# cwerner/deadtrees

Measured on AMD Instinct MI355X. Metric: 512x512 RGB tiles/sec (train fwd+bwd), higher is better.
Workload: dtype f32; 1 GPU; configs[1]: reference U-Net (smp Unet/resnet34 topology) fp32 train step, batch 32/GPU, 512x512x3 tiles, GDICE+FOCAL, clip 0.5, Adam 3e-4; global_batch=32, tile=512, parallelism=dp1

## Files before the change

deadtrees_amd/csrc/common.h:

```cpp
#pragma once
#include <hip/hip_runtime.h>
#include <stdint.h>
#include <stdio.h>
#include <stdarg.h>
#include <type_traits>

#include "../../include/deadtrees_hip.h"

typedef float f32x16 __attribute__((ext_vector_type(16)));
typedef float f32x4 __attribute__((ext_vector_type(4)));
typedef float f32x2 __attribute__((ext_vector_type(2)));
typedef unsigned u32x2 __attribute__((ext_vector_type(2)));
typedef unsigned u32x4 __attribute__((ext_vector_type(4)));
typedef __bf16 bf16x8 __attribute__((ext_vector_type(8)));
typedef __bf16 bf16x4 __attribute__((ext_vector_type(4)));
typedef __bf16 bf16x2 __attribute__((ext_vector_type(2)));
typedef const void __attribute__((address_space(1)))* dt_gptr;
typedef void __attribute__((address_space(3)))* dt_lptr;

void dt_set_error(const char* fmt, ...);

#define DT_REQUIRE(cond, ...)            \
  do {                                   \
    if (!(cond)) {                       \
// ... 7 lines not shown
    hipError_t e__ = hipGetLastError();                                          \
    if (e__ != hipSuccess) {                                                     \
      dt_set_error("%s:%d launch failed: %s", __FILE__, __LINE__, hipGetErrorString(e__)); \
      return DT_EHIP;                                                            \
    }                                                                            \
  } while (0)

static inline int dt_cdiv(int64_t a, int64_t b) { return (int)((a + b - 1) / b); }

__device__ __forceinline__ float wave_sum(float v) {
#pragma unroll
  for (int o = 32; o > 0; o >>= 1) v += __shfl_xor(v, o, 64);
  return v;
}
__device__ __forceinline__ double wave_sum_d(double v) {
#pragma unroll
  for (int o = 32; o > 0; o >>= 1) v += __shfl_xor(v, o, 64);
  return v;
}

int dt_reduce_rows_launch(const float* in, float* out, int planes, int P, int N, int RB, hipStream_t st);
static inline int dt_reduce_rows_out(int P, int RB) { return (P + RB - 1) / RB; }

template <int K, int N, class F>
__device__ __forceinline__ void dt_static_for(F&& f) {
  if constexpr (K < N) {
    f(std::integral_constant<int, K>{});
    dt_static_for<K + 1, N>(f);
  }
}

__device__ __forceinline__ void dt_dma16(const void* g, void* l) {
  __builtin_amdgcn_global_load_lds((dt_gptr)g, (dt_lptr)l, 16, 0, 0);
}

__device__ __forceinline__ unsigned xcd_remap(unsigned id, unsigned n) {
  const unsigned q = n >> 3, r = n & 7u, xcd = id & 7u, idx = id >> 3;
  const unsigned base = xcd < r ? xcd * (q + 1) : r * (q + 1) + (xcd - r) * q;
  return base + idx;
}

extern "C" int dt_conv2d_n16_supported(const dt_conv_desc* d);
int dt_conv2d_n16_launch(const dt_conv_desc* d, const float* src0, const float* w, float* out, float* stats,
                         const float* in_scale, const float* in_shift, hipStream_t st,
                         const dt_bn_bwd_fuse* fuse = nullptr);
extern "C" int dt_conv2d_wgrad_n16_supported(const dt_conv_desc* d);
// ... 15 lines not shown
```

deadtrees_amd/csrc/conv_bf16.hip:

```cpp
#include "conv_host.h"


#include "conv_bf16.h"

#define BF_CK 32
#define BF_TF_MAXC 512
#define BF_NARROW_CIN 32

template <int KS, int STRIDE, int TW, int TPX>
struct BfGeom {
  static constexpr int TH = TPX / TW;
  static constexpr int LS = (KS == 1) ? 1 : STRIDE;
  static constexpr int GS = (KS == 1) ? STRIDE : 1;
  static constexpr int HALO_H = (TH - 1) * LS + KS;
  static constexpr int HALO_W = (TW - 1) * LS + KS;
  static constexpr int TAPS = KS * KS;
};

template <int KS, int STRIDE, int TW, int TN, int CK, int MT, bool TF>
__global__ __launch_bounds__(256, (KS == 3 && STRIDE == 2) ? 1 : 2) void conv_fwd_bf16_kernel(const ConvBfArgs a) {
  constexpr int TPX = 128 * MT;
  using G = BfGeom<KS, STRIDE, TW, TPX>;
  constexpr int BF_PITCH = CK + 8, SEG = CK / 8, ROWS_IT = 256 / SEG;
  constexpr int NT = TN / 32;
// ... 1091 lines not shown
             "wgrad_bf16: ksize/stride (%d,%d) unsupported", d->ksize, d->stride);
  DT_REQUIRE((d->C0 & 7) == 0 && (d->C1 & 7) == 0 && (d->Cout & 7) == 0, "wgrad_bf16: channels must be multiples of 8");
  DT_REQUIRE(d->mode0 >= 0 && d->mode0 <= 1, "wgrad_bf16: mode0");
  return dt_conv_validate_out(d, "wgrad_bf16");
}

extern "C" size_t dt_conv2d_wgrad_bf16_workspace(const dt_conv_desc* d) {
  if (wb_validate(d) != DT_OK) return 0;
  int tw, ks, T, cib, cob;
  wb_cfg(d, &tw, &ks, &T, &cib, &cob);
  const size_t E = (size_t)d->ksize * d->ksize * (d->C0 + d->C1) * d->Cout;
  size_t need = (size_t)ks * E * sizeof(float);
  if (dt_wgrad_bf16_narrow_supported(d)) {
    const size_t n3 = dt_wgrad_bf16_narrow_workspace(d);
    if (n3 > need) need = n3;
  }
  if (wb_use_dma() && dt_wgrad_bf16_dma_supported(d)) {
    const size_t n2 = dt_wgrad_bf16_dma_workspace(d);
    if (n2 > need) need = n2;
  }
  return need;
}

__global__ __launch_bounds__(256) void wgrad_bf16_final_kernel(const float* __restrict__ ws, float* __restrict__ dw,
                                                               int parts, int64_t E) {
  __shared__ f32x4 sh[256];
  const int q = threadIdx.x & 15, rl = threadIdx.x >> 4;
  const int64_t E4 = E >> 2, e4 = (int64_t)blockIdx.x * 16 + q;
  f32x4 a0 = {0.f, 0.f, 0.f, 0.f}, a1 = a0, a2 = a0, a3 = a0;
  if (e4 < E4) {
    const f32x4* src = reinterpret_cast<const f32x4*>(ws) + e4;
    int p = rl;
    for (; p + 48 < parts; p += 64) {
      const f32x4 v0 = src[(size_t)p * E4], v1 = src[(size_t)(p + 16) * E4];
      const f32x4 v2 = src[(size_t)(p + 32) * E4], v3 = src[(size_t)(p + 48) * E4];
      a0 += v0; a1 += v1; a2 += v2; a3 += v3;
    }
    for (; p < parts; p += 16) a0 += src[(size_t)p * E4];
  }
  sh[threadIdx.x] = (a0 + a1) + (a2 + a3);
  __syncthreads();
  if (rl == 0 && e4 < E4) {
    double t[4] = {0.0, 0.0, 0.0, 0.0};
    for (int i = 0; i < 16; ++i) {
      const f32x4 v = sh[i * 16 + q];
#pragma unroll
      for (int k = 0; k < 4; ++k) t[k] += (double)v[k];
    }
    reinterpret_cast<f32x4*>(dw)[e4] = f32x4{(float)t[0], (float)t[1], (float)t[2], (float)t[3]};
  }
}

template <int KS, int STRIDE, int TW>
static int wb_launch(const WgradBfArgs& a, int grid, hipStream_t st) {
  const bool narrow = a.C0 + a.C1 <= 32 && a.Cout <= 32;
  if (narrow) {
    if constexpr (KS == 3 && STRIDE == 1) {
      if (a.in_scale != nullptr)
        hipLaunchKernelGGL((conv_wgrad_bf16_kernel<KS, STRIDE, TW, true, 32>), dim3(grid), dim3(256), 0, st, a);
      else
        hipLaunchKernelGGL((conv_wgrad_bf16_kernel<KS, STRIDE, TW, false, 32>), dim3(grid), dim3(256), 0, st, a);
      DT_LAUNCH_CHECK();
      return DT_OK;
    }
  }
  if (a.in_scale != nullptr)
    hipLaunchKernelGGL((conv_wgrad_bf16_kernel<KS, STRIDE, TW, true, 64>), dim3(grid), dim3(256), 0, st, a);
  else
    hipLaunchKernelGGL((conv_wgrad_bf16_kernel<KS, STRIDE, TW, false, 64>), dim3(grid), dim3(256), 0, st, a);
  DT_LAUNCH_CHECK();
  return DT_OK;
}

extern "C" int dt_conv2d_wgrad_bf16(const dt_conv_desc* d, const void* src0, const void* src1, const void* dy,
                                    float* dw_hwio, float* workspace, size_t workspace_bytes, const float* in_scale,
                                    const float* in_shift, void* stream) {
  int rc = wb_validate(d);
  if (rc != DT_OK) return rc;
  DT_REQUIRE(src0 && dy && dw_hwio && workspace, "wgrad_bf16: null pointer");
  DT_REQUIRE(d->C1 == 0 || src1, "wgrad_bf16: src1 missing");
  DT_REQUIRE((in_scale == nullptr) == (in_shift == nullptr), "wgrad_bf16: in_scale/in_shift must come together");
  DT_REQUIRE(workspace_bytes >= dt_conv2d_wgrad_bf16_workspace(d), "wgrad_bf16: workspace too small");
  hipStream_t st = (hipStream_t)stream;
  const int64_t E = (int64_t)d->ksize * d->ksize * (d->C0 + d->C1) * d->Cout;
  if (dt_wgrad_bf16_narrow_supported(d)) {
    const int parts = dt_wgrad_bf16_narrow_launch(d, src0, dy, workspace, in_scale, in_shift, st);
    if (parts < 0) return parts;
    hipLaunchKernelGGL(wgrad_bf16_final_kernel, dim3((unsigned)((E / 4 + 15) / 16)), dim3(256), 0, st, workspace, dw_hwio,
                       parts, E);
    DT_LAUNCH_CHECK();
    return DT_OK;
  }
  if (in_scale == nullptr && wb_use_dma() && dt_wgrad_bf16_dma_supported(d)) {
    const int parts = dt_wgrad_bf16_dma_launch(d, src0, src1, dy, workspace, st);
    if (parts < 0) return parts;
    hipLaunchKernelGGL(wgrad_bf16_final_kernel, dim3((unsigned)((E / 4 + 15) / 16)), dim3(256), 0, st, workspace, dw_hwio,
                       parts, E);
    DT_LAUNCH_CHECK();
    return DT_OK;
  }
  WgradBfArgs a;
  int tw;
  wb_cfg(d, &tw, &a.ksplit, &a.T, &a.ci_blocks, &a.co_blocks);
  a.src0 = (const __bf16*)src0; a.src1 = (const __bf16*)src1; a.dy = (const __bf16*)dy; a.ws = workspace;
  a.in_scale = in_scale; a.in_shift = in_shift;
  a.B = d->B; a.Hin = d->Hin; a.Win = d->Win; a.C0 = d->C0; a.C1 = d->C1; a.mode0 = d->mode0;
  a.Ho = d->Ho; a.Wo = d->Wo; a.Cout = d->Cout; a.pad = d->pad;
  a.tiles_x = dt_cdiv(d->Wo, tw); a.tiles_y = dt_cdiv(d->Ho, 128 / tw);
  const int grid = a.ci_blocks * a.co_blocks * a.ksplit * (d->ksize == 4 ? 2 : 1);
  if (d->ksize == 4) {
    DT_REQUIRE(in_scale == nullptr, "wgrad_bf16: the stem takes no input transform");
    hipLaunchKernelGGL((conv_wgrad_bf16_kernel<4, 1, 32, false, 32>), dim3(grid), dim3(256), 0, st, a);
    DT_LAUNCH_CHECK();
    rc = DT_OK;
  } else if (d->ksize == 3 && d->stride == 1) rc = tw == 32 ? wb_launch<3, 1, 32>(a, grid, st) : wb_launch<3, 1, 16>(a, grid, st);
  else if (d->ksize == 3) rc = tw == 32 ? wb_launch<3, 2, 32>(a, grid, st) : wb_launch<3, 2, 16>(a, grid, st);
  else if (d->stride == 2) rc = tw == 32 ? wb_launch<1, 2, 32>(a, grid, st) : wb_launch<1, 2, 16>(a, grid, st);
  else rc = tw == 32 ? wb_launch<1, 1, 32>(a, grid, st) : wb_launch<1, 1, 16>(a, grid, st);
  if (rc != DT_OK) return rc;
  DT_REQUIRE((E & 3) == 0, "wgrad_bf16: weight tensor size must be a multiple of 4");
  const int64_t g = (E / 4 + 15) / 16;
  hipLaunchKernelGGL(wgrad_bf16_final_kernel, dim3((unsigned)g), dim3(256), 0, st, workspace, dw_hwio, a.ksplit, E);
  DT_LAUNCH_CHECK();
  return DT_OK;
}
```

deadtrees_amd/csrc/conv_wgrad.hip:

```cpp
#include "conv_host.h"

struct WgradArgs {
  const float* src0;
  const float* src1;
  const float* in_scale;
  const float* in_shift;
  const float* dy;
  const __bf16* dy_bf16;
  float* ws;
  int B, Hin, Win, C0, C1, mode0;
  int Ho, Wo, Cout, pad;
  int tiles_x, tiles_y, T;
  int ci_blocks, co_blocks, ksplit;
};

template <int KS, int STRIDE, int TW, int TPX>
struct WGeom {
  static constexpr int TH = TPX / TW;
  static constexpr int LS = (KS == 1) ? 1 : STRIDE;
  static constexpr int GS = (KS == 1) ? STRIDE : 1;
  static constexpr int HALO_H = (TH - 1) * LS + KS;
  static constexpr int HALO_W = (TW - 1) * LS + KS;
  static constexpr int TAPS = KS * KS;
};
// ... 132 lines not shown
#pragma unroll
        for (int t = 0; t < G::TAPS; ++t) {
          const int kh = t / KS, kw = t % KS;
          const float av = lx[xbase + ((yy * WK * G::LS + kh) * G::HALO_W + 2 * j * G::LS + kw) * CIW];
          acc[t] = __builtin_amdgcn_mfma_f32_32x32x2f32(av, bv, acc[t], 0, 0, 0);
        }
      }
    }
  }
  const int part = ks * WK + wk;
  const int co = co0 + wco * 32 + r;
  if (co < a.Cout) {
#pragma unroll
    for (int t = 0; t < G::TAPS; ++t) {
#pragma unroll
      for (int i = 0; i < 16; ++i) {
        const int ci = ci0 + wci * 32 + (i & 3) + 8 * (i >> 2) + 4 * s;
        if (ci < Cin) a.ws[(((size_t)part * G::TAPS + t) * Cin + ci) * a.Cout + co] = acc[t][i];
      }
    }
  }
}

__global__ __launch_bounds__(256) void wgrad_reduce_kernel(const float* __restrict__ ws, float* __restrict__ dw,
                                                           int parts, int64_t E) {
  const int64_t stride = (int64_t)gridDim.x * blockDim.x;
  for (int64_t e = (int64_t)blockIdx.x * blockDim.x + threadIdx.x; e < E; e += stride) {
    double s = 0.0;
    for (int p = 0; p < parts; ++p) s += (double)ws[(size_t)p * E + e];
    dw[e] = (float)s;
  }
}

#define STEM_TW 32
#define STEM_TH 4
__global__ __launch_bounds__(256, 2) void conv_wgrad_stem_kernel(const WgradArgs a) {
  constexpr int KS = 7, TW = STEM_TW, TH = STEM_TH;
  constexpr int HALO_H = (TH - 1) * 2 + KS, HALO_W = (TW - 1) * 2 + KS;
  constexpr int X_ELEMS = HALO_H * HALO_W * 4 + 32;
  constexpr int COW = 64;
  __shared__ __attribute__((aligned(16))) float lds[X_ELEMS + TH * TW * COW];
  float* lx = lds;
  float* ly = lds + X_ELEMS;
  const int tid = threadIdx.x, lane = tid & 63, wave = tid >> 6;
  const int s = lane >> 5, r = lane & 31;
  const int cob = blockIdx.x % a.co_blocks, ks = blockIdx.x / a.co_blocks;
  const int co0 = cob * COW;
  const int wco = wave & 1, wk = wave >> 1;
  f32x16 acc[KS];
#pragma unroll
  for (int t = 0; t < KS; ++t)
#pragma unroll
    for (int i = 0; i < 16; ++i) acc[t][i] = 0.f;
  const int Cin = a.C0;
// ... 194 lines not shown
  a.src0 = src0; a.src1 = src1; a.dy = dy; a.ws = workspace; a.in_scale = in_scale; a.in_shift = in_shift;
  a.dy_bf16 = (const __bf16*)dy_bf16;
  a.B = d->B; a.Hin = d->Hin; a.Win = d->Win; a.C0 = d->C0; a.C1 = d->C1; a.mode0 = d->mode0;
  a.Ho = d->Ho; a.Wo = d->Wo; a.Cout = d->Cout; a.pad = d->pad;
  a.tiles_x = c.tiles_x; a.tiles_y = c.tiles_y; a.T = c.T;
  a.ci_blocks = c.ci_blocks; a.co_blocks = c.co_blocks; a.ksplit = c.ksplit;
  hipStream_t st = (hipStream_t)stream;
  const int grid = c.ci_blocks * c.co_blocks * c.ksplit;
  if (c.narrow) {
    rc = dt_wgrad_n16_launch(d, src0, dy, workspace, in_scale, in_shift, st);
  } else if (c.stem) {
    hipLaunchKernelGGL(conv_wgrad_stem_kernel, dim3(grid), dim3(256), 0, st, a);
    DT_LAUNCH_CHECK();
  } else if (d->ksize == 3 && d->stride == 1) {
    rc = c.tw == 32 ? wg_dispatch<3, 1, 32>(a, c, grid, st) : wg_dispatch<3, 1, 16>(a, c, grid, st);
  } else if (d->ksize == 3 && d->stride == 2) {
    rc = c.tw == 32 ? wg_launch<3, 2, 32, 64, 1, 2>(a, grid, st) : wg_launch<3, 2, 16, 64, 1, 2>(a, grid, st);
  } else if (d->stride == 2) {
    rc = c.tw == 32 ? wg_dispatch<1, 2, 32>(a, c, grid, st) : wg_dispatch<1, 2, 16>(a, c, grid, st);
  } else {
    rc = c.tw == 32 ? wg_dispatch<1, 1, 32>(a, c, grid, st) : wg_dispatch<1, 1, 16>(a, c, grid, st);
  }
  if (rc != DT_OK) return rc;
  const float* slabs = workspace;
  int nslabs = c.parts;
  if (c.parts2 != c.parts) {
    float* stage = workspace + (size_t)c.parts * E;
    rc = dt_reduce_rows_launch(workspace, stage, 1, c.parts, (int)E, c.rb, st);
    if (rc != DT_OK) return rc;
    slabs = stage;
    nslabs = c.parts2;
  }
  const int g = dt_ew_grid(E, 256 * 8);
  hipLaunchKernelGGL(wgrad_reduce_kernel, dim3((unsigned)g), dim3(256), 0, st, slabs, dw, nslabs, E);
  DT_LAUNCH_CHECK();
  return DT_OK;
}

extern "C" int dt_conv2d_wgrad(const dt_conv_desc* d, const float* src0, const float* src1, const float* dy,
                               float* dw, float* workspace, size_t workspace_bytes, const float* in_scale,
                               const float* in_shift, void* stream) {
  return wgrad_impl(d, src0, src1, dy, nullptr, dw, workspace, workspace_bytes, in_scale, in_shift, stream);
}

extern "C" int dt_conv2d_wgrad_stem_dy_bf16(const dt_conv_desc* d, const float* src0, const void* dy_bf16, float* dw,
                                            float* workspace, size_t workspace_bytes, void* stream) {
  DT_REQUIRE(d && d->ksize == 7 && dy_bf16, "wgrad_stem_dy_bf16: 7x7 stem only");
  return wgrad_impl(d, src0, nullptr, reinterpret_cast<const float*>(dy_bf16), dy_bf16, dw, workspace, workspace_bytes,
                    nullptr, nullptr, stream);
}
```

deadtrees_amd/csrc/conv_wino_wgrad.hip:

```cpp
#include "conv_host.h"


#define WW_BUF 8192
#define WW_TF_MAXC 512
#define WW_OOB 0x80000000u
#define WW_MAX_WGS 256

struct WinoWgArgs {
  const float* src0;
  const float* src1;
  const float* dy;
  const float* in_scale;
  const float* in_shift;
  float* ws;
  int B, Hin, Win, C0, C1, mode0, Cout;
  int tiles_x, tiles_y, T;
  int ci_blocks, co_blocks, ksplit, cps;
  unsigned bytes0, bytes1, dybytes, wsbytes;
};

template <bool TF, bool CO32 = false>
__global__ __launch_bounds__(256, 1) void conv3x3_wino_wgrad_kernel(const WinoWgArgs a) {
  __shared__ __attribute__((aligned(1024))) float lds[4 * WW_BUF + (TF ? 2 * WW_TF_MAXC : 4)];
  float* Vb = lds;
// ... 251 lines not shown
  for (int c = 0; c < a.cps; c += 2) {
    asm volatile("s_waitcnt lgkmcnt(0)\n\ts_barrier" ::: "memory");
    step(S0{});
    asm volatile("s_waitcnt lgkmcnt(0)\n\ts_barrier" ::: "memory");
    step(S1{});
  }

  const __amdgpu_buffer_rsrc_t rsw = __builtin_amdgcn_make_buffer_rsrc((void*)a.ws, 0, a.wsbytes, 0x00020000);
  const unsigned lane_base = (unsigned)(((32 * wm + 4 * kh) * 64 + (CO32 ? 0 : 32 * wn) + r) * 4);
  const int wg_base = ((CO32 ? 2 * split + wn : split) * nblocks + blk) * (16 * 4096 * 4);
#pragma unroll
  for (int p = 0; p < 16; ++p) {
#pragma unroll
    for (int i = 0; i < 16; ++i) {
      const int m = (i & 3) + 8 * (i >> 2);
      const float v = acc[p][i];
      __builtin_amdgcn_raw_buffer_store_b32(__builtin_bit_cast(unsigned, v), rsw, lane_base,
                                            wg_base + (p * 4096 + m * 64) * 4, 0);
    }
    __builtin_amdgcn_sched_barrier(0);
  }
}

__global__ __launch_bounds__(256) void wino_wgrad_reduce_kernel(const float* __restrict__ ws, float* __restrict__ ws2,
                                                                int64_t n4, int ksplit, int rb) {
  const int64_t i = (int64_t)blockIdx.x * 256 + threadIdx.x;
  if (i >= n4) return;
  const int g = blockIdx.y;
  const int s0 = g * rb, s1 = s0 + rb < ksplit ? s0 + rb : ksplit;
  f32x4 s = {0.f, 0.f, 0.f, 0.f};
  for (int k = s0; k < s1; ++k) s += *reinterpret_cast<const f32x4*>(ws + ((int64_t)k * n4 + i) * 4);
  *reinterpret_cast<f32x4*>(ws2 + ((int64_t)g * n4 + i) * 4) = s;
}

__global__ __launch_bounds__(256) void wino_wgrad_final_kernel(const float* __restrict__ ws, float* __restrict__ dw,
                                                               int parts, int ci_blocks, int co_blocks, int Cin,
                                                               int Cout) {
  const int blk = blockIdx.y;
  const int e = blockIdx.x * 256 + threadIdx.x;
  const int ci = (blk / co_blocks) * 64 + (e >> 6), co = (blk % co_blocks) * 64 + (e & 63);
  if (co >= Cout) return;
  const int64_t n = (int64_t)ci_blocks * co_blocks * 16 * 4096;
  float u[16];
#pragma unroll
  for (int p = 0; p < 16; ++p) u[p] = 0.f;
  for (int k = 0; k < parts; ++k) {
    const float* src = ws + (int64_t)k * n + (int64_t)blk * 16 * 4096 + e;
#pragma unroll
    for (int p = 0; p < 16; ++p) u[p] += src[p * 4096];
  }
  float tt[12];
#pragma unroll
  for (int j = 0; j < 4; ++j) {
    tt[0 + j] = u[0 + j] + 0.5f * (u[4 + j] + u[8 + j]);
    tt[4 + j] = 0.5f * (u[4 + j] - u[8 + j]);
    tt[8 + j] = 0.5f * (u[4 + j] + u[8 + j]) + u[12 + j];
  }
#pragma unroll
  for (int i = 0; i < 3; ++i) {
    const float g0 = tt[4 * i + 0] + 0.5f * (tt[4 * i + 1] + tt[4 * i + 2]);
    const float g1 = 0.5f * (tt[4 * i + 1] - tt[4 * i + 2]);
    const float g2 = 0.5f * (tt[4 * i + 1] + tt[4 * i + 2]) + tt[4 * i + 3];
    dw[((size_t)(3 * i + 0) * Cin + ci) * Cout + co] = g0;
    dw[((size_t)(3 * i + 1) * Cin + ci) * Cout + co] = g1;
    dw[((size_t)(3 * i + 2) * Cin + ci) * Cout + co] = g2;
  }
}

struct WwCfg {
  int tiles_x, tiles_y, T, ci_blocks, co_blocks, ksplit, cps, rb, groups, parts;
};

// ... 48 lines not shown
  DT_REQUIRE((in_scale == nullptr) == (in_shift == nullptr), "wgrad_winograd: in_scale/in_shift must come together");
  DT_REQUIRE(workspace_bytes >= dt_conv2d_wgrad_winograd_workspace(d), "wgrad_winograd: workspace too small");
  const WwCfg c = ww_cfg(d);
  const size_t slab = (size_t)c.ci_blocks * c.co_blocks * 16 * 4096 * 4;
  DT_REQUIRE(slab * c.parts < 0x100000000ull, "wgrad_winograd: workspace beyond 4 GiB");
  WinoWgArgs a;
  a.src0 = src0; a.src1 = src1; a.dy = dy; a.in_scale = in_scale; a.in_shift = in_shift; a.ws = workspace;
  a.B = d->B; a.Hin = d->Hin; a.Win = d->Win; a.C0 = d->C0; a.C1 = d->C1; a.mode0 = d->mode0; a.Cout = d->Cout;
  a.tiles_x = c.tiles_x; a.tiles_y = c.tiles_y; a.T = c.T;
  a.ci_blocks = c.ci_blocks; a.co_blocks = c.co_blocks; a.ksplit = c.ksplit; a.cps = c.cps;
  const size_t px0 = (size_t)d->B * (d->mode0 ? (d->Hin / 2) * (size_t)(d->Win / 2) : (size_t)d->Hin * d->Win);
  a.bytes0 = (unsigned)(px0 * d->C0 * 4);
  a.bytes1 = (unsigned)((size_t)d->B * d->Hin * d->Win * d->C1 * 4);
  a.dybytes = (unsigned)((size_t)d->B * d->Ho * d->Wo * d->Cout * 4);
  a.wsbytes = (unsigned)(slab * c.parts);
  hipStream_t st = (hipStream_t)stream;
  dim3 g((unsigned)(c.ci_blocks * c.co_blocks * c.ksplit)), blk(256);
  if (d->Cout == 32) {
    if (in_scale != nullptr) hipLaunchKernelGGL((conv3x3_wino_wgrad_kernel<true, true>), g, blk, 0, st, a);
    else hipLaunchKernelGGL((conv3x3_wino_wgrad_kernel<false, true>), g, blk, 0, st, a);
  } else if (in_scale != nullptr) hipLaunchKernelGGL((conv3x3_wino_wgrad_kernel<true>), g, blk, 0, st, a);
  else hipLaunchKernelGGL((conv3x3_wino_wgrad_kernel<false>), g, blk, 0, st, a);
  DT_LAUNCH_CHECK();
  const float* parts_src = workspace;
  int parts = c.parts;
  if (c.rb > 1) {
    float* ws2 = workspace + slab / 4 * c.parts;
    const int64_t n4 = (int64_t)(slab / 16);
    hipLaunchKernelGGL(wino_wgrad_reduce_kernel, dim3((unsigned)dt_cdiv(n4, 256), (unsigned)c.groups), dim3(256), 0, st,
                       workspace, ws2, n4, c.parts, c.rb);
    DT_LAUNCH_CHECK();
    parts_src = ws2;
    parts = c.groups;
  }
  hipLaunchKernelGGL(wino_wgrad_final_kernel, dim3(16, (unsigned)(c.ci_blocks * c.co_blocks)), dim3(256), 0, st, parts_src,
                     dw_hwio, parts, c.ci_blocks, c.co_blocks, d->C0 + d->C1, d->Cout);
  DT_LAUNCH_CHECK();
  return DT_OK;
}
```

deadtrees_amd/csrc/elementwise.hip:

```cpp
#include "conv_host.h"
#include "views.h"

#include <math.h>

__device__ __forceinline__ void relu_mask_from_y(f32x4& g, const f32x4 yv, const f32x4 asc, const f32x4 ash) {
  const f32x4 a = yv * asc + ash;
#pragma unroll
  for (int k = 0; k < 4; ++k) g[k] = a[k] > 0.f ? g[k] : 0.f;
}
__device__ __forceinline__ void bnb_sums(const f32x4 g, const f32x4 yv, const f32x4 mu, const f32x4 is, f32x4& sg, f32x4& sx) {
  sg += g;
  sx += g * ((yv - mu) * is);
}
__device__ __forceinline__ void bnb_masked_sums(f32x4 g, const f32x4 yv, const f32x4 asc, const f32x4 ash, const f32x4 mu,
                                                const f32x4 is, f32x4& sg, f32x4& sx) {
  relu_mask_from_y(g, yv, asc, ash);
  bnb_sums(g, yv, mu, is, sg, sx);
}

__device__ __forceinline__ void bnb_store_partial_rows(const f32x4 sg, const f32x4 sx, int L, int cq, int row, int P, int C4,
                                                       float* __restrict__ red) {
  __shared__ f32x4 sh[2][256];
  const int t = threadIdx.x, rl = t / L, RL = 256 / L;
  sh[0][t] = sg;
// ... 36 lines not shown
    }
    for (; r < r1; r += RL) a0 += src[(size_t)r * N4 + cq];
  }
  sh[t] = (a0 + a1) + (a2 + a3);
  __syncthreads();
  if (rl == 0 && cq < N4) {
    f32x4 s = sh[q];
    for (int i = 1; i < RL; ++i) s += sh[i * Q + q];
    reinterpret_cast<f32x4*>(out)[((size_t)blockIdx.z * PB + blockIdx.y) * N4 + cq] = s;
  }
}

int dt_reduce_rows_launch(const float* in, float* out, int planes, int P, int N, int RB, hipStream_t st) {
  const int N4 = N / 4;
  int Q = 64;
  while (Q > N4) Q >>= 1;
  if (Q < 1) Q = 1;
  dim3 grid(dt_cdiv(N4, Q), dt_cdiv(P, RB), planes);
  hipLaunchKernelGGL(reduce_rows_kernel, grid, dim3(256), 0, st, in, out, P, N, RB, Q);
  DT_LAUNCH_CHECK();
  return DT_OK;
}

__global__ __launch_bounds__(256) void bn_finalize_kernel(const float* __restrict__ stats, int P, int C,
                                                          double count, const float* __restrict__ gamma,
                                                          const float* __restrict__ beta, float eps,
                                                          float momentum, const float* __restrict__ momentum_dev,
                                                          float* running_mean,
                                                          float* running_var, float* mean, float* invstd,
                                                          float* scale, float* shift) {
  __shared__ double red[2][16][17];
  if (momentum_dev) momentum = momentum_dev[0];
  const int cl = threadIdx.x & 15, rl = threadIdx.x >> 4;
  const int c = blockIdx.x * 16 + cl;
  double s1 = 0.0, s2 = 0.0;
  if (c < C) {
    double u1 = 0.0, u2 = 0.0, v1 = 0.0, v2 = 0.0, w1 = 0.0, w2 = 0.0;
    int p = rl;
    for (; p + 48 < P; p += 64) {
      const float a0 = stats[(size_t)p * C + c], a1 = stats[(size_t)(p + 16) * C + c];
      const float a2 = stats[(size_t)(p + 32) * C + c], a3 = stats[(size_t)(p + 48) * C + c];
      const float b0 = stats[((size_t)P + p) * C + c], b1 = stats[((size_t)P + p + 16) * C + c];
      const float b2 = stats[((size_t)P + p + 32) * C + c], b3 = stats[((size_t)P + p + 48) * C + c];
      s1 += (double)a0; u1 += (double)a1; v1 += (double)a2; w1 += (double)a3;
      s2 += (double)b0; u2 += (double)b1; v2 += (double)b2; w2 += (double)b3;
    }
    for (; p < P; p += 16) {
      s1 += (double)stats[(size_t)p * C + c];
      s2 += (double)stats[((size_t)P + p) * C + c];
    }
    s1 = (s1 + u1) + (v1 + w1);
    s2 = (s2 + u2) + (v2 + w2);
  }
  red[0][rl][cl] = s1;
  red[1][rl][cl] = s2;
  __syncthreads();
  if (rl == 0 && c < C) {
    double t1 = 0.0, t2 = 0.0;
    for (int i = 0; i < 16; ++i) {
      t1 += red[0][i][cl];
      t2 += red[1][i][cl];
    }
    const double m = t1 / count;
    double var = t2 / count - m * m;
    if (var < 0.0) var = 0.0;
    const double is = 1.0 / sqrt(var + (double)eps);
    mean[c] = (float)m;
    invstd[c] = (float)is;
    const float sc = gamma[c] * (float)is;
    scale[c] = sc;
    shift[c] = beta[c] - (float)m * sc;
    if (running_mean) {
      const double unb = count > 1.0 ? var * count / (count - 1.0) : var;
      running_mean[c] = (1.f - momentum) * running_mean[c] + momentum * (float)m;
      running_var[c] = (1.f - momentum) * running_var[c] + momentum * (float)unb;
    }
  }
}

#define BN_STAGE1_MIN_ROWS 256
#define BN_STAGE1_RB 64

extern "C" int64_t dt_bn_stats_floats(int P, int C) {
  return (int64_t)2 * P * C + (int64_t)2 * dt_reduce_rows_out(P, BN_STAGE1_RB) * C;
}

static int bn_finalize_launch(float* stats, int P, int C, double count, const float* gamma, const float* beta, float eps,
                              float momentum, const float* momentum_dev, float* running_mean, float* running_var,
                              float* mean, float* invstd, float* scale, float* shift, void* stream) {
  DT_REQUIRE(stats && gamma && beta && mean && invstd && scale && shift && P > 0 && C > 0 && count > 0,
             "bn_finalize: bad args");
  if (P > BN_STAGE1_MIN_ROWS && (C & 3) == 0) {
    const int PB = dt_reduce_rows_out(P, BN_STAGE1_RB);
    float* scratch = stats + (size_t)2 * P * C;
    int rc = dt_reduce_rows_launch(stats, scratch, 2, P, C, BN_STAGE1_RB, (hipStream_t)stream);
    if (rc != DT_OK) return rc;
    stats = scratch;
    P = PB;
  }
  hipLaunchKernelGGL(bn_finalize_kernel, dim3(dt_cdiv(C, 16)), dim3(256), 0, (hipStream_t)stream, stats, P, C,
                     count, gamma, beta, eps, momentum, momentum_dev, running_mean, running_var, mean, invstd, scale,
                     shift);
  DT_LAUNCH_CHECK();
  return DT_OK;
}

extern "C" int dt_bn_finalize(float* stats, int P, int C, double count, const float* gamma,
                              const float* beta, float eps, float momentum, float* running_mean,
                              float* running_var, float* mean, float* invstd, float* scale, float* shift,
                              void* stream) {
  return bn_finalize_launch(stats, P, C, count, gamma, beta, eps, momentum, nullptr, running_mean, running_var, mean,
                            invstd, scale, shift, stream);
}

extern "C" int dt_bn_finalize_dev(float* stats, int P, int C, double count, const float* gamma, const float* beta,
                                  float eps, const float* momentum_dev, float* running_mean, float* running_var,
                                  float* mean, float* invstd, float* scale, float* shift, void* stream) {
  DT_REQUIRE(momentum_dev && running_mean && running_var, "bn_finalize_dev: momentum_dev and running statistics required");
  return bn_finalize_launch(stats, P, C, count, gamma, beta, eps, 0.f, momentum_dev, running_mean, running_var, mean,
                            invstd, scale, shift, stream);
}

__global__ void bn_eval_affine_kernel(const float* gamma, const float* beta, const float* rm, const float* rv,
// ... 234 lines not shown
    bnb_sums(g0, y[o0], mu, is, sg0, sx0);
  }
  bnb_store_partial_rows(sg0 + sg1, sx0 + sx1, Q, cq, blockIdx.y, P, C4, red);
}

extern "C" int dt_bn_bwd_reduce(const float* dout, const float* out_act, const float* y, const float* mean,
                                const float* invstd, const float* act_scale, const float* act_shift, float* red,
                                int64_t n_pix, int C, void* stream) {
  DT_REQUIRE(dout && y && mean && invstd && red && n_pix > 0 && C > 0 && (C & 3) == 0, "bn_bwd_reduce: bad args");
  const int C4 = C / 4;
  int Q = 64;
  while (Q > C4) Q >>= 1;
  DT_REQUIRE(C4 % Q == 0, "bn_bwd_reduce: C/4 must be a power of two or a multiple of 64 (C=%d)", C);
  const int P = dt_bn_bwd_rows(n_pix, C);
  hipLaunchKernelGGL(bn_bwd_reduce_kernel, dim3(C4 / Q, P), dim3(256), 0, (hipStream_t)stream, (const f32x4*)dout,
                     (const f32x4*)out_act, (const f32x4*)y, mean, invstd, act_scale, act_shift, red, n_pix, C4, Q, P,
                     bnb_rb(n_pix));
  DT_LAUNCH_CHECK();
  return DT_OK;
}

__global__ __launch_bounds__(256) void bn_bwd_sums_kernel(const float* __restrict__ red, int P, int C,
                                                          float* __restrict__ dgamma, float* __restrict__ dbeta) {
  __shared__ double sh[2][16][17];
  const int cl = threadIdx.x & 15, rl = threadIdx.x >> 4;
  const int c = blockIdx.x * 16 + cl;
  double s1 = 0.0, s2 = 0.0;
  if (c < C) {
    double u1 = 0.0, u2 = 0.0, v1 = 0.0, v2 = 0.0, w1 = 0.0, w2 = 0.0;
    int p = rl;
    for (; p + 48 < P; p += 64) {
      const float a0 = red[(size_t)p * C + c], a1 = red[(size_t)(p + 16) * C + c];
      const float a2 = red[(size_t)(p + 32) * C + c], a3 = red[(size_t)(p + 48) * C + c];
      const float b0 = red[((size_t)P + p) * C + c], b1 = red[((size_t)P + p + 16) * C + c];
      const float b2 = red[((size_t)P + p + 32) * C + c], b3 = red[((size_t)P + p + 48) * C + c];
      s1 += (double)a0; u1 += (double)a1; v1 += (double)a2; w1 += (double)a3;
      s2 += (double)b0; u2 += (double)b1; v2 += (double)b2; w2 += (double)b3;
    }
    for (; p < P; p += 16) {
      s1 += (double)red[(size_t)p * C + c];
      s2 += (double)red[((size_t)P + p) * C + c];
    }
    s1 = (s1 + u1) + (v1 + w1);
    s2 = (s2 + u2) + (v2 + w2);
  }
  sh[0][rl][cl] = s1;
  sh[1][rl][cl] = s2;
  __syncthreads();
  if (rl == 0 && c < C) {
    double t1 = 0.0, t2 = 0.0;
    for (int i = 0; i < 16; ++i) {
      t1 += sh[0][i][cl];
      t2 += sh[1][i][cl];
    }
    dbeta[c] = (float)t1;
    dgamma[c] = (float)t2;
  }
}

int dt_bn_bwd_finish_sums(float* red, int P, int C, float* dgamma, float* dbeta, hipStream_t st) {
  if (P > BN_STAGE1_MIN_ROWS) {
    const int PB = dt_reduce_rows_out(P, BN_STAGE1_RB);
    float* scratch = red + (size_t)2 * P * C;
    int rc = dt_reduce_rows_launch(red, scratch, 2, P, C, BN_STAGE1_RB, st);
    if (rc != DT_OK) return rc;
    red = scratch;
    P = PB;
  }
  hipLaunchKernelGGL(bn_bwd_sums_kernel, dim3(dt_cdiv(C, 16)), dim3(256), 0, st, red, P, C, dgamma, dbeta);
  DT_LAUNCH_CHECK();
  return DT_OK;
}

#define BN_LD(p) __builtin_nontemporal_load(p)
__global__ __launch_bounds__(256) void bn_bwd_apply_kernel(
    const f32x4* __restrict__ dout, const f32x4* __restrict__ out_act, const f32x4* __restrict__ y,
    const float* __restrict__ mean, const float* __restrict__ invstd, const float* __restrict__ gamma,
    const float* __restrict__ dgamma, const float* __restrict__ dbeta, const float* __restrict__ act_scale,
    const float* __restrict__ act_shift, f32x4* __restrict__ dy, f32x4* __restrict__ dres, int dres_acc, int64_t n4,
    int C4, float inv_count) {
  const int64_t stride = (int64_t)gridDim.x * blockDim.x;
  const int64_t i0 = (int64_t)blockIdx.x * blockDim.x + threadIdx.x;
  const bool fixed = (stride % C4) == 0;
  f32x4 asc = {1.f, 1.f, 1.f, 1.f}, ash = {0.f, 0.f, 0.f, 0.f}, mu, is, gi, kb, kg;
  auto load_coef = [&](int c4) {
    if (act_scale) {
      asc = reinterpret_cast<const f32x4*>(act_scale)[c4];
      ash = reinterpret_cast<const f32x4*>(act_shift)[c4];
    }
    mu = reinterpret_cast<const f32x4*>(mean)[c4];
    is = reinterpret_cast<const f32x4*>(invstd)[c4];
    gi = reinterpret_cast<const f32x4*>(gamma)[c4] * is;
// ... 548 lines not shown
```

Baseline: 835.8 tiles/s.

## Collapse two-stage partial-sum reductions into single-pass wide reductions for wgrad and BN

Replaces the two-launch reductions (reduce-rows stage then final) for weight-gradient partial slabs and BN stats with single kernels that spread the partial-sum axis across more threads per output. The generic fp32 wgrad path now uses the shared vectorized final kernel instead of a scalar per-element loop plus a staging pass. The winograd wgrad final kernel gets an XCD-remapped, split-slab variant. The BN column-sum kernels now use 4 channels per block with 256 rows in parallel, and the stage-1 threshold rises so most layers skip the extra launch. This removes launches and intermediate traffic, at the cost of changing summation order, which may slightly alter results.

```diff
diff --git a/deadtrees_amd/csrc/common.h b/deadtrees_amd/csrc/common.h
--- a/deadtrees_amd/csrc/common.h
+++ b/deadtrees_amd/csrc/common.h
@@ -53,6 +53,8 @@
 int dt_reduce_rows_launch(const float* in, float* out, int planes, int P, int N, int RB, hipStream_t st);
 static inline int dt_reduce_rows_out(int P, int RB) { return (P + RB - 1) / RB; }
 
+int dt_wgrad_final_launch(const float* ws, float* dw, int parts, int64_t E, hipStream_t st);
+
 template <int K, int N, class F>
 __device__ __forceinline__ void dt_static_for(F&& f) {
   if constexpr (K < N) {
diff --git a/deadtrees_amd/csrc/conv_bf16.hip b/deadtrees_amd/csrc/conv_bf16.hip
--- a/deadtrees_amd/csrc/conv_bf16.hip
+++ b/deadtrees_amd/csrc/conv_bf16.hip
@@ -1137,35 +1137,6 @@
   return need;
 }
 
-__global__ __launch_bounds__(256) void wgrad_bf16_final_kernel(const float* __restrict__ ws, float* __restrict__ dw,
-                                                               int parts, int64_t E) {
-  __shared__ f32x4 sh[256];
-  const int q = threadIdx.x & 15, rl = threadIdx.x >> 4;
-  const int64_t E4 = E >> 2, e4 = (int64_t)blockIdx.x * 16 + q;
-  f32x4 a0 = {0.f, 0.f, 0.f, 0.f}, a1 = a0, a2 = a0, a3 = a0;
-  if (e4 < E4) {
-    const f32x4* src = reinterpret_cast<const f32x4*>(ws) + e4;
-    int p = rl;
-    for (; p + 48 < parts; p += 64) {
-      const f32x4 v0 = src[(size_t)p * E4], v1 = src[(size_t)(p + 16) * E4];
-      const f32x4 v2 = src[(size_t)(p + 32) * E4], v3 = src[(size_t)(p + 48) * E4];
-      a0 += v0; a1 += v1; a2 += v2; a3 += v3;
-    }
-    for (; p < parts; p += 16) a0 += src[(size_t)p * E4];
-  }
-  sh[threadIdx.x] = (a0 + a1) + (a2 + a3);
-  __syncthreads();
-  if (rl == 0 && e4 < E4) {
-    double t[4] = {0.0, 0.0, 0.0, 0.0};
-    for (int i = 0; i < 16; ++i) {
-      const f32x4 v = sh[i * 16 + q];
-#pragma unroll
-      for (int k = 0; k < 4; ++k) t[k] += (double)v[k];
-    }
-    reinterpret_cast<f32x4*>(dw)[e4] = f32x4{(float)t[0], (float)t[1], (float)t[2], (float)t[3]};
-  }
-}
-
 template <int KS, int STRIDE, int TW>
 static int wb_launch(const WgradBfArgs& a, int grid, hipStream_t st) {
   const bool narrow = a.C0 + a.C1 <= 32 && a.Cout <= 32;
@@ -1201,18 +1172,12 @@
   if (dt_wgrad_bf16_narrow_supported(d)) {
     const int parts = dt_wgrad_bf16_narrow_launch(d, src0, dy, workspace, in_scale, in_shift, st);
     if (parts < 0) return parts;
-    hipLaunchKernelGGL(wgrad_bf16_final_kernel, dim3((unsigned)((E / 4 + 15) / 16)), dim3(256), 0, st, workspace, dw_hwio,
-                       parts, E);
-    DT_LAUNCH_CHECK();
-    return DT_OK;
+    return dt_wgrad_final_launch(workspace, dw_hwio, parts, E, st);
   }
   if (in_scale == nullptr && wb_use_dma() && dt_wgrad_bf16_dma_supported(d)) {
     const int parts = dt_wgrad_bf16_dma_launch(d, src0, src1, dy, workspace, st);
     if (parts < 0) return parts;
-    hipLaunchKernelGGL(wgrad_bf16_final_kernel, dim3((unsigned)((E / 4 + 15) / 16)), dim3(256), 0, st, workspace, dw_hwio,
-                       parts, E);
-    DT_LAUNCH_CHECK();
-    return DT_OK;
+    return dt_wgrad_final_launch(workspace, dw_hwio, parts, E, st);
   }
   WgradBfArgs a;
   int tw;
@@ -1233,9 +1198,5 @@
   else if (d->stride == 2) rc = tw == 32 ? wb_launch<1, 2, 32>(a, grid, st) : wb_launch<1, 2, 16>(a, grid, st);
   else rc = tw == 32 ? wb_launch<1, 1, 32>(a, grid, st) : wb_launch<1, 1, 16>(a, grid, st);
   if (rc != DT_OK) return rc;
-  DT_REQUIRE((E & 3) == 0, "wgrad_bf16: weight tensor size must be a multiple of 4");
-  const int64_t g = (E / 4 + 15) / 16;
-  hipLaunchKernelGGL(wgrad_bf16_final_kernel, dim3((unsigned)g), dim3(256), 0, st, workspace, dw_hwio, a.ksplit, E);
-  DT_LAUNCH_CHECK();
-  return DT_OK;
-}
+  return dt_wgrad_final_launch(workspace, dw_hwio, a.ksplit, E, st);
+}
diff --git a/deadtrees_amd/csrc/conv_wgrad.hip b/deadtrees_amd/csrc/conv_wgrad.hip
--- a/deadtrees_amd/csrc/conv_wgrad.hip
+++ b/deadtrees_amd/csrc/conv_wgrad.hip
@@ -178,14 +178,40 @@
   }
 }
 
-__global__ __launch_bounds__(256) void wgrad_reduce_kernel(const float* __restrict__ ws, float* __restrict__ dw,
-                                                           int parts, int64_t E) {
-  const int64_t stride = (int64_t)gridDim.x * blockDim.x;
-  for (int64_t e = (int64_t)blockIdx.x * blockDim.x + threadIdx.x; e < E; e += stride) {
-    double s = 0.0;
-    for (int p = 0; p < parts; ++p) s += (double)ws[(size_t)p * E + e];
-    dw[e] = (float)s;
-  }
+__global__ __launch_bounds__(256) void wgrad_final_kernel(const float* __restrict__ ws, float* __restrict__ dw, int parts,
+                                                          int64_t E) {
+  __shared__ f32x4 sh[256];
+  const int q = threadIdx.x & 15, rl = threadIdx.x >> 4;
+  const int64_t E4 = E >> 2, e4 = (int64_t)blockIdx.x * 16 + q;
+  f32x4 a0 = {0.f, 0.f, 0.f, 0.f}, a1 = a0, a2 = a0, a3 = a0;
+  if (e4 < E4) {
+    const f32x4* src = reinterpret_cast<const f32x4*>(ws) + e4;
+    int p = rl;
+    for (; p + 48 < parts; p += 64) {
+      const f32x4 v0 = src[(size_t)p * E4], v1 = src[(size_t)(p + 16) * E4];
+      const f32x4 v2 = src[(size_t)(p + 32) * E4], v3 = src[(size_t)(p + 48) * E4];
+      a0 += v0; a1 += v1; a2 += v2; a3 += v3;
+    }
+    for (; p < parts; p += 16) a0 += src[(size_t)p * E4];
+  }
+  sh[threadIdx.x] = (a0 + a1) + (a2 + a3);
+  __syncthreads();
+  if (rl == 0 && e4 < E4) {
+    double t[4] = {0.0, 0.0, 0.0, 0.0};
+    for (int i = 0; i < 16; ++i) {
+      const f32x4 v = sh[i * 16 + q];
+#pragma unroll
+      for (int k = 0; k < 4; ++k) t[k] += (double)v[k];
+    }
+    reinterpret_cast<f32x4*>(dw)[e4] = f32x4{(float)t[0], (float)t[1], (float)t[2], (float)t[3]};
+  }
+}
+
+int dt_wgrad_final_launch(const float* ws, float* dw, int parts, int64_t E, hipStream_t st) {
+  DT_REQUIRE((E & 3) == 0, "wgrad: weight tensor size must be a multiple of 4");
+  hipLaunchKernelGGL(wgrad_final_kernel, dim3((unsigned)((E / 4 + 15) / 16)), dim3(256), 0, st, ws, dw, parts, E);
+  DT_LAUNCH_CHECK();
+  return DT_OK;
 }
 
 #define STEM_TW 32
@@ -426,19 +452,7 @@
     rc = c.tw == 32 ? wg_dispatch<1, 1, 32>(a, c, grid, st) : wg_dispatch<1, 1, 16>(a, c, grid, st);
   }
   if (rc != DT_OK) return rc;
-  const float* slabs = workspace;
-  int nslabs = c.parts;
-  if (c.parts2 != c.parts) {
-    float* stage = workspace + (size_t)c.parts * E;
-    rc = dt_reduce_rows_launch(workspace, stage, 1, c.parts, (int)E, c.rb, st);
-    if (rc != DT_OK) return rc;
-    slabs = stage;
-    nslabs = c.parts2;
-  }
-  const int g = dt_ew_grid(E, 256 * 8);
-  hipLaunchKernelGGL(wgrad_reduce_kernel, dim3((unsigned)g), dim3(256), 0, st, slabs, dw, nslabs, E);
-  DT_LAUNCH_CHECK();
-  return DT_OK;
+  return dt_wgrad_final_launch(workspace, dw, c.parts, E, st);
 }
 
 extern "C" int dt_conv2d_wgrad(const dt_conv_desc* d, const float* src0, const float* src1, const float* dy,
diff --git a/deadtrees_amd/csrc/conv_wino_wgrad.hip b/deadtrees_amd/csrc/conv_wino_wgrad.hip
--- a/deadtrees_amd/csrc/conv_wino_wgrad.hip
+++ b/deadtrees_amd/csrc/conv_wino_wgrad.hip
@@ -297,32 +297,50 @@
   }
 }
 
-__global__ __launch_bounds__(256) void wino_wgrad_reduce_kernel(const float* __restrict__ ws, float* __restrict__ ws2,
-                                                                int64_t n4, int ksplit, int rb) {
-  const int64_t i = (int64_t)blockIdx.x * 256 + threadIdx.x;
-  if (i >= n4) return;
-  const int g = blockIdx.y;
-  const int s0 = g * rb, s1 = s0 + rb < ksplit ? s0 + rb : ksplit;
-  f32x4 s = {0.f, 0.f, 0.f, 0.f};
-  for (int k = s0; k < s1; ++k) s += *reinterpret_cast<const f32x4*>(ws + ((int64_t)k * n4 + i) * 4);
-  *reinterpret_cast<f32x4*>(ws2 + ((int64_t)g * n4 + i) * 4) = s;
-}
-
+template <int SL>
 __global__ __launch_bounds__(256) void wino_wgrad_final_kernel(const float* __restrict__ ws, float* __restrict__ dw,
-                                                               int parts, int ci_blocks, int co_blocks, int Cin,
+                                                               int parts, int nblocks, int co_blocks, int Cin,
                                                                int Cout) {
-  const int blk = blockIdx.y;
-  const int e = blockIdx.x * 256 + threadIdx.x;
-  const int ci = (blk / co_blocks) * 64 + (e >> 6), co = (blk % co_blocks) * 64 + (e & 63);
-  if (co >= Cout) return;
-  const int64_t n = (int64_t)ci_blocks * co_blocks * 16 * 4096;
+  constexpr int EL = 64 / SL, QN = EL / 4;
+  __shared__ f32x4 sh[SL][16][QN];
+  const int t = threadIdx.x, q = t % QN, pos = (t / QN) & 15, sl = t / (16 * QN);
+  const int wg = (int)xcd_remap(blockIdx.x, gridDim.x);
+  const int blk = wg / (4096 / EL), e0 = (wg % (4096 / EL)) * EL;
+  const int ci = (blk / co_blocks) * 64 + (e0 >> 6), co0 = (blk % co_blocks) * 64 + (e0 & 63);
+  const bool live = co0 + 4 * q < Cout;
+  f32x4 acc[4];
+#pragma unroll
+  for (int k = 0; k < 4; ++k) acc[k] = f32x4{0.f, 0.f, 0.f, 0.f};
+  if (live) {
+    const int64_t n4 = (int64_t)nblocks * 16 * 1024;
+    const f32x4* src = reinterpret_cast<const f32x4*>(ws) + ((int64_t)blk * 16 + pos) * 1024 + (e0 >> 2) + q;
+    int p = sl;
+    auto rounds = [&](auto n) {
+      constexpr int N = decltype(n)::value;
+      for (; p + (N - 1) * SL < parts; p += N * SL) {
+        f32x4 v[N];
+#pragma unroll
+        for (int k = 0; k < N; ++k) v[k] = src[(int64_t)(p + k * SL) * n4];
+#pragma unroll
+        for (int k = 0; k < N; ++k) acc[k & 3] += v[k];
+      }
+    };
+    rounds(std::integral_constant<int, 16>{});
+    rounds(std::integral_constant<int, 4>{});
+    rounds(std::integral_constant<int, 1>{});
+  }
+  sh[sl][pos][q] = (acc[0] + acc[1]) + (acc[2] + acc[3]);
+  __syncthreads();
+  const int co = co0 + t;
+  if (t >= EL || co >= Cout) return;
+  const float* shf = reinterpret_cast<const float*>(sh);
   float u[16];
 #pragma unroll
-  for (int p = 0; p < 16; ++p) u[p] = 0.f;
-  for (int k = 0; k < parts; ++k) {
-    const float* src = ws + (int64_t)k * n + (int64_t)blk * 16 * 4096 + e;
-#pragma unroll
-    for (int p = 0; p < 16; ++p) u[p] += src[p * 4096];
+  for (int p = 0; p < 16; ++p) {
+    double s = 0.0;
+#pragma unroll
+    for (int l = 0; l < SL; ++l) s += (double)shf[(l * 16 + p) * EL + t];
+    u[p] = (float)s;
   }
   float tt[12];
 #pragma unroll
@@ -417,19 +435,13 @@
   } else if (in_scale != nullptr) hipLaunchKernelGGL((conv3x3_wino_wgrad_kernel<true>), g, blk, 0, st, a);
   else hipLaunchKernelGGL((conv3x3_wino_wgrad_kernel<false>), g, blk, 0, st, a);
   DT_LAUNCH_CHECK();
-  const float* parts_src = workspace;
-  int parts = c.parts;
-  if (c.rb > 1) {
-    float* ws2 = workspace + slab / 4 * c.parts;
-    const int64_t n4 = (int64_t)(slab / 16);
-    hipLaunchKernelGGL(wino_wgrad_reduce_kernel, dim3((unsigned)dt_cdiv(n4, 256), (unsigned)c.groups), dim3(256), 0, st,
-                       workspace, ws2, n4, c.parts, c.rb);
-    DT_LAUNCH_CHECK();
-    parts_src = ws2;
-    parts = c.groups;
-  }
-  hipLaunchKernelGGL(wino_wgrad_final_kernel, dim3(16, (unsigned)(c.ci_blocks * c.co_blocks)), dim3(256), 0, st, parts_src,
-                     dw_hwio, parts, c.ci_blocks, c.co_blocks, d->C0 + d->C1, d->Cout);
+  const int nblocks = c.ci_blocks * c.co_blocks;
+  if (nblocks <= 8)
+    hipLaunchKernelGGL(wino_wgrad_final_kernel<4>, dim3((unsigned)(nblocks * 256)), dim3(256), 0, st, workspace, dw_hwio,
+                       c.parts, nblocks, c.co_blocks, d->C0 + d->C1, d->Cout);
+  else
+    hipLaunchKernelGGL(wino_wgrad_final_kernel<1>, dim3((unsigned)(nblocks * 64)), dim3(256), 0, st, workspace, dw_hwio,
+                       c.parts, nblocks, c.co_blocks, d->C0 + d->C1, d->Cout);
   DT_LAUNCH_CHECK();
   return DT_OK;
 }
diff --git a/deadtrees_amd/csrc/elementwise.hip b/deadtrees_amd/csrc/elementwise.hip
--- a/deadtrees_amd/csrc/elementwise.hip
+++ b/deadtrees_amd/csrc/elementwise.hip
@@ -82,6 +82,55 @@
   return DT_OK;
 }
 
+__device__ __forceinline__ f32x4 bn_row_quad(const float* __restrict__ rows, size_t row, int C, int c0, bool vec) {
+  if (vec) return *reinterpret_cast<const f32x4*>(rows + row * C + c0);
+  f32x4 v = {0.f, 0.f, 0.f, 0.f};
+#pragma unroll
+  for (int k = 0; k < 4; ++k)
+    if (c0 + k < C) v[k] = rows[row * C + c0 + k];
+  return v;
+}
+
+__device__ __forceinline__ void bn_column_sums(const float* __restrict__ rows, int P, int C, double& t1, double& t2) {
+  __shared__ double sh[4][8];
+  const int t = threadIdx.x, c0 = 4 * blockIdx.x;
+  const bool vec = (C & 3) == 0;
+  double s[8] = {0.0, 0.0, 0.0, 0.0, 0.0, 0.0, 0.0, 0.0};
+  int p = t;
+  auto rounds = [&](auto n) {
+    constexpr int N = decltype(n)::value;
+    for (; p + (N - 1) * 256 < P; p += N * 256) {
+      f32x4 a[N], b[N];
+#pragma unroll
+      for (int k = 0; k < N; ++k) {
+        a[k] = bn_row_quad(rows, (size_t)p + k * 256, C, c0, vec);
+        b[k] = bn_row_quad(rows, (size_t)P + p + k * 256, C, c0, vec);
+      }
+#pragma unroll
+      for (int k = 0; k < N; ++k)
+#pragma unroll
+        for (int j = 0; j < 4; ++j) {
+          s[j] += (double)a[k][j];
+          s[4 + j] += (double)b[k][j];
+        }
+    }
+  };
+  rounds(std::integral_constant<int, 8>{});
+  rounds(std::integral_constant<int, 2>{});
+  rounds(std::integral_constant<int, 1>{});
+#pragma unroll
+  for (int j = 0; j < 8; ++j) s[j] = wave_sum_d(s[j]);
+  if ((t & 63) == 0) {
+#pragma unroll
+    for (int j = 0; j < 8; ++j) sh[t >> 6][j] = s[j];
+  }
+  __syncthreads();
+  if (t < 4) {
+    t1 = (sh[0][t] + sh[1][t]) + (sh[2][t] + sh[3][t]);
+    t2 = (sh[0][4 + t] + sh[1][4 + t]) + (sh[2][4 + t] + sh[3][4 + t]);
+  }
+}
+
 __global__ __launch_bounds__(256) void bn_finalize_kernel(const float* __restrict__ stats, int P, int C,
                                                           double count, const float* __restrict__ gamma,
                                                           const float* __restrict__ beta, float eps,
@@ -89,60 +138,53 @@
                                                           float* running_mean,
                                                           float* running_var, float* mean, float* invstd,
                                                           float* scale, float* shift) {
-  __shared__ double red[2][16][17];
   if (momentum_dev) momentum = momentum_dev[0];
-  const int cl = threadIdx.x & 15, rl = threadIdx.x >> 4;
-  const int c = blockIdx.x * 16 + cl;
-  double s1 = 0.0, s2 = 0.0;
-  if (c < C) {
-    double u1 = 0.0, u2 = 0.0, v1 = 0.0, v2 = 0.0, w1 = 0.0, w2 = 0.0;
-    int p = rl;
-    for (; p + 48 < P; p += 64) {
-      const float a0 = stats[(size_t)p * C + c], a1 = stats[(size_t)(p + 16) * C + c];
-      const float a2 = stats[(size_t)(p + 32) * C + c], a3 = stats[(size_t)(p + 48) * C + c];
-      const float b0 = stats[((size_t)P + p) * C + c], b1 = stats[((size_t)P + p + 16) * C + c];
-      const float b2 = stats[((size_t)P + p + 32) * C + c], b3 = stats[((size_t)P + p + 48) * C + c];
-      s1 += (double)a0; u1 += (double)a1; v1 += (double)a2; w1 += (double)a3;
-      s2 += (double)b0; u2 += (double)b1; v2 += (double)b2; w2 += (double)b3;
-    }
-    for (; p < P; p += 16) {
-      s1 += (double)stats[(size_t)p * C + c];
-      s2 += (double)stats[((size_t)P + p) * C + c];
-    }
-    s1 = (s1 + u1) + (v1 + w1);
-    s2 = (s2 + u2) + (v2 + w2);
-  }
-  red[0][rl][cl] = s1;
-  red[1][rl][cl] = s2;
-  __syncthreads();
-  if (rl == 0 && c < C) {
-    double t1 = 0.0, t2 = 0.0;
-    for (int i = 0; i < 16; ++i) {
-      t1 += red[0][i][cl];
-      t2 += red[1][i][cl];
-    }
+  const int c = 4 * blockIdx.x + threadIdx.x;
+  const bool mine = threadIdx.x < 4 && c < C;
+  float ga = 0.f, be = 0.f, rm = 0.f, rv = 0.f;
+  if (mine) {
+    ga = gamma[c];
+    be = beta[c];
+    if (running_mean) {
+      rm = running_mean[c];
+      rv = running_var[c];
+    }
+  }
+  double t1 = 0.0, t2 = 0.0;
+  bn_column_sums(stats, P, C, t1, t2);
+  if (mine) {
     const double m = t1 / count;
     double var = t2 / count - m * m;
     if (var < 0.0) var = 0.0;
     const double is = 1.0 / sqrt(var + (double)eps);
     mean[c] = (float)m;
     invstd[c] = (float)is;
-    const float sc = gamma[c] * (float)is;
+    const float sc = ga * (float)is;
     scale[c] = sc;
-    shift[c] = beta[c] - (float)m * sc;
+    shift[c] = be - (float)m * sc;
     if (running_mean) {
       const double unb = count > 1.0 ? var * count / (count - 1.0) : var;
-      running_mean[c] = (1.f - momentum) * running_mean[c] + momentum * (float)m;
-      running_var[c] = (1.f - momentum) * running_var[c] + momentum * (float)unb;
-    }
-  }
-}
-
-#define BN_STAGE1_MIN_ROWS 256
+      running_mean[c] = (1.f - momentum) * rm + momentum * (float)m;
+      running_var[c] = (1.f - momentum) * rv + momentum * (float)unb;
+    }
+  }
+}
+
+#define BN_STAGE1_MIN_ROWS 2048
 #define BN_STAGE1_RB 64
 
 extern "C" int64_t dt_bn_stats_floats(int P, int C) {
   return (int64_t)2 * P * C + (int64_t)2 * dt_reduce_rows_out(P, BN_STAGE1_RB) * C;
+}
+
+static int bn_stage1(float*& rows, int& P, int C, hipStream_t st) {
+  if (P <= BN_STAGE1_MIN_ROWS || (C & 3) != 0) return DT_OK;
+  const int PB = dt_reduce_rows_out(P, BN_STAGE1_RB);
+  float* scratch = rows + (size_t)2 * P * C;
+  DT_TRY(dt_reduce_rows_launch(rows, scratch, 2, P, C, BN_STAGE1_RB, st));
+  rows = scratch;
+  P = PB;
+  return DT_OK;
 }
 
 static int bn_finalize_launch(float* stats, int P, int C, double count, const float* gamma, const float* beta, float eps,
@@ -150,15 +192,8 @@
                               float* mean, float* invstd, float* scale, float* shift, void* stream) {
   DT_REQUIRE(stats && gamma && beta && mean && invstd && scale && shift && P > 0 && C > 0 && count > 0,
              "bn_finalize: bad args");
-  if (P > BN_STAGE1_MIN_ROWS && (C & 3) == 0) {
-    const int PB = dt_reduce_rows_out(P, BN_STAGE1_RB);
-    float* scratch = stats + (size_t)2 * P * C;
-    int rc = dt_reduce_rows_launch(stats, scratch, 2, P, C, BN_STAGE1_RB, (hipStream_t)stream);
-    if (rc != DT_OK) return rc;
-    stats = scratch;
-    P = PB;
-  }
-  hipLaunchKernelGGL(bn_finalize_kernel, dim3(dt_cdiv(C, 16)), dim3(256), 0, (hipStream_t)stream, stats, P, C,
+  DT_TRY(bn_stage1(stats, P, C, (hipStream_t)stream));
+  hipLaunchKernelGGL(bn_finalize_kernel, dim3(dt_cdiv(C, 4)), dim3(256), 0, (hipStream_t)stream, stats, P, C,
                      count, gamma, beta, eps, momentum, momentum_dev, running_mean, running_var, mean, invstd, scale,
                      shift);
   DT_LAUNCH_CHECK();
@@ -439,52 +474,18 @@
 
 __global__ __launch_bounds__(256) void bn_bwd_sums_kernel(const float* __restrict__ red, int P, int C,
                                                           float* __restrict__ dgamma, float* __restrict__ dbeta) {
-  __shared__ double sh[2][16][17];
-  const int cl = threadIdx.x & 15, rl = threadIdx.x >> 4;
-  const int c = blockIdx.x * 16 + cl;
-  double s1 = 0.0, s2 = 0.0;
-  if (c < C) {
-    double u1 = 0.0, u2 = 0.0, v1 = 0.0, v2 = 0.0, w1 = 0.0, w2 = 0.0;
-    int p = rl;
-    for (; p + 48 < P; p += 64) {
-      const float a0 = red[(size_t)p * C + c], a1 = red[(size_t)(p + 16) * C + c];
-      const float a2 = red[(size_t)(p + 32) * C + c], a3 = red[(size_t)(p + 48) * C + c];
-      const float b0 = red[((size_t)P + p) * C + c], b1 = red[((size_t)P + p + 16) * C + c];
-      const float b2 = red[((size_t)P + p + 32) * C + c], b3 = red[((size_t)P + p + 48) * C + c];
-      s1 += (double)a0; u1 += (double)a1; v1 += (double)a2; w1 += (double)a3;
-      s2 += (double)b0; u2 += (double)b1; v2 += (double)b2; w2 += (double)b3;
-    }
-    for (; p < P; p += 16) {
-      s1 += (double)red[(size_t)p * C + c];
-      s2 += (double)red[((size_t)P + p) * C + c];
-    }
-    s1 = (s1 + u1) + (v1 + w1);
-    s2 = (s2 + u2) + (v2 + w2);
-  }
-  sh[0][rl][cl] = s1;
-  sh[1][rl][cl] = s2;
-  __syncthreads();
-  if (rl == 0 && c < C) {
-    double t1 = 0.0, t2 = 0.0;
-    for (int i = 0; i < 16; ++i) {
-      t1 += sh[0][i][cl];
-      t2 += sh[1][i][cl];
-    }
+  double t1 = 0.0, t2 = 0.0;
+  bn_column_sums(red, P, C, t1, t2);
+  const int c = 4 * blockIdx.x + threadIdx.x;
+  if (threadIdx.x < 4 && c < C) {
     dbeta[c] = (float)t1;
     dgamma[c] = (float)t2;
   }
 }
 
 int dt_bn_bwd_finish_sums(float* red, int P, int C, float* dgamma, float* dbeta, hipStream_t st) {
-  if (P > BN_STAGE1_MIN_ROWS) {
-    const int PB = dt_reduce_rows_out(P, BN_STAGE1_RB);
-    float* scratch = red + (size_t)2 * P * C;
-    int rc = dt_reduce_rows_launch(red, scratch, 2, P, C, BN_STAGE1_RB, st);
-    if (rc != DT_OK) return rc;
-    red = scratch;
-    P = PB;
-  }
-  hipLaunchKernelGGL(bn_bwd_sums_kernel, dim3(dt_cdiv(C, 16)), dim3(256), 0, st, red, P, C, dgamma, dbeta);
+  DT_TRY(bn_stage1(red, P, C, st));
+  hipLaunchKernelGGL(bn_bwd_sums_kernel, dim3(dt_cdiv(C, 4)), dim3(256), 0, st, red, P, C, dgamma, dbeta);
   DT_LAUNCH_CHECK();
   return DT_OK;
 }
```

Measured after the change: 839.7 tiles/s (median of 6 runs). No clear change (+0.5%).
